# amzn/MXFusion

Hardware: AMD Instinct MI355X
Metric: ELBO-steps/sec + RBF Gram GB/s, SVGP N=65k D=8 M=1024, 1->8 MI355X (higher is better)
Workload: dtype f32; 1 GPU; SVGPRegression RBF-ARD N=65536 Q=8 M=1024, 32 MC samples (latent-input model), StochasticVariationalInference step = draw + ELBO + reverse mode + grad all-reduce + Adam; samples_per_gpu=32, parallelism=mc-samples sharded x1, 1 RCCL all-reduce of the flat gradient/step, core_precision=float64 (M x M factorisations), streaming float32

## Files before the change

mxfusion_amd/csrc/gemm_split.hip:

```cpp
#include "common.h"
#include "internal.h"
#include "split_device.h"

namespace {

typedef __bf16 bf16x8 __attribute__((ext_vector_type(8)));

constexpr int SBM = 128, SBN = 128, SNT = 256;

template <int NP>
__global__ __launch_bounds__(256) void split_planes_kernel(int64_t R, int64_t K, const float* __restrict__ X, int64_t ld,
                                                           unsigned short* __restrict__ P, int64_t pstride, const unsigned* __restrict__ maxbits) {
    __shared__ float tile[64][68];
    const int tid = threadIdx.x;
    const int64_t r0 = (int64_t)blockIdx.y * 64, k0 = (int64_t)blockIdx.x * 64;
    for (int it = 0; it < 4; ++it) {
        const int row = it * 16 + (tid >> 4), c = (tid & 15) * 4;
        const int64_t r = r0 + row, k = k0 + c;
        float4 v = make_float4(0.f, 0.f, 0.f, 0.f);
        if (r < R) {
            if (k + 3 < K && ((ld & 3) == 0) && (((uintptr_t)X & 15) == 0)) v = *reinterpret_cast<const float4*>(X + r * ld + k);
            else {
                if (k + 0 < K) v.x = X[r * ld + k + 0];
                if (k + 1 < K) v.y = X[r * ld + k + 1];
                if (k + 2 < K) v.z = X[r * ld + k + 2];
                if (k + 3 < K) v.w = X[r * ld + k + 3];
            }
        }
        tile[row][c + 0] = v.x; tile[row][c + 1] = v.y; tile[row][c + 2] = v.z; tile[row][c + 3] = v.w;
    }
    __syncthreads();
    const int row = tid & 63, kbl = tid >> 6;
    const int64_t r = r0 + row, kb = k0 / 16 + kbl;
    const int64_t Kp16 = (K + 15) / 16;
    if (r >= R || kb >= Kp16) return;
    unsigned short h[16], m[16], l[16];
    const float sc = (NP == 2 && maxbits) ? scale_from_maxbits(maxbits[0]) : 1.f;
#pragma unroll
    for (int j = 0; j < 16; ++j) {
        const float x = tile[row][kbl * 16 + j];
        if (NP == 2) {
            const float xs = x * sc;
            const _Float16 fh = (_Float16)xs;
            const _Float16 fl = (_Float16)(xs - (float)fh);
            h[j] = __builtin_bit_cast(unsigned short, fh); m[j] = __builtin_bit_cast(unsigned short, fl); l[j] = 0;
            continue;
        }
        const __bf16 bh = (__bf16)x;
        const float r1 = x - (float)bh;
        const __bf16 bm = (__bf16)r1;
        const float r2 = r1 - (float)bm;
        const __bf16 bl = (__bf16)r2;
        h[j] = __builtin_bit_cast(unsigned short, bh); m[j] = __builtin_bit_cast(unsigned short, bm); l[j] = __builtin_bit_cast(unsigned short, bl);
    }
    const int64_t off = (kb * R + r) * 16;
    auto put = [&](unsigned short* dst, const unsigned short (&v)[16]) {
        u32x4 a, b;
#pragma unroll
        for (int j = 0; j < 4; ++j) { a[j] = (unsigned)v[2 * j] | ((unsigned)v[2 * j + 1] << 16); b[j] = (unsigned)v[8 + 2 * j] | ((unsigned)v[8 + 2 * j + 1] << 16); }
        *reinterpret_cast<u32x4*>(dst) = a;
        *reinterpret_cast<u32x4*>(dst + 8) = b;
    };
    put(P + off, h);
    put(P + pstride + off, m);
    if (NP == 3) put(P + 2 * pstride + off, l);
}

__global__ __launch_bounds__(256) void maxabs_kernel(int64_t n, int64_t K, int64_t ld, const float* __restrict__ x, unsigned* __restrict__ out) {
    __shared__ unsigned wm[4];
    unsigned m = 0;
    for (int64_t i = (int64_t)blockIdx.x * 256 + threadIdx.x; i < n; i += (int64_t)gridDim.x * 256) {
        const unsigned b = __builtin_bit_cast(unsigned, x[(i / K) * ld + i % K]) & 0x7fffffffu;
        m = b > m ? b : m;
    }
    for (int o = 32; o > 0; o >>= 1) { const unsigned t = (unsigned)__shfl_xor((int)m, o); m = t > m ? t : m; }
    if ((threadIdx.x & 63) == 0) wm[threadIdx.x >> 6] = m;
    __syncthreads();
    if (threadIdx.x == 0) {
        for (int w = 1; w < 4; ++w) m = wm[w] > m ? wm[w] : m;
        atomicMax(out, m);
    }
}

__global__ __launch_bounds__(256) void maxabs_flat_kernel(int64_t n4, const uint4* __restrict__ x, unsigned* __restrict__ out) {
    __shared__ unsigned wm[4];
    unsigned m = 0;
    for (int64_t i = (int64_t)blockIdx.x * 256 + threadIdx.x; i < n4; i += (int64_t)gridDim.x * 256) {
        const uint4 v = x[i];
        const unsigned a = v.x & 0x7fffffffu, b = v.y & 0x7fffffffu, c = v.z & 0x7fffffffu, d = v.w & 0x7fffffffu;
        const unsigned ab = a > b ? a : b, cd = c > d ? c : d, q = ab > cd ? ab : cd;
        m = q > m ? q : m;
    }
    for (int o = 32; o > 0; o >>= 1) { const unsigned t = (unsigned)__shfl_xor((int)m, o); m = t > m ? t : m; }
    if ((threadIdx.x & 63) == 0) wm[threadIdx.x >> 6] = m;
    __syncthreads();
    if (threadIdx.x == 0) {
        for (int w = 1; w < 4; ++w) m = wm[w] > m ? wm[w] : m;
        atomicMax(out, m);
    }
}

struct SplitArgs {
    const unsigned short* A; const unsigned short* B; float* C;
    int64_t M, N, K16;
    int64_t pA, pB, ldc;
    float alpha, beta;
    int splitk, lower_only, atomic, nprod, use_dma;
    int c_blk;
    int64_t kchunk;
    int64_t tm, tn, ntiles, nwg;
    const float* ad0; int pow0;
    const unsigned* maxbits;
    const unsigned* maxbits2;
    unsigned* sync; int sync_n, sync_period, sync_slots;
    unsigned* maxout;
    unsigned short* Cp; int64_t pC;
    int64_t rot_div;
    int a_lower;
    int pair;
    unsigned short* Ct; int64_t pCt;
    const float* avec; float* Upart;
    int cp_nt;
};

template <bool DMA, int NP>
__global__ __launch_bounds__(SNT, (NP == 2 && !DMA) ? 4 : 3) void gemm_split_kernel(SplitArgs g) {
    constexpr int NST = (DMA && NP == 2) ? 3 : 2;
    __shared__ u32x4 smem[NST][2][NP][256];
    const int tid = threadIdx.x, lane = tid & 63, wave = tid >> 6;
    const int wm = (wave >> 1) * 64, wn = (wave & 1) * 64;
    const int64_t wid = xcd_run_item((int64_t)blockIdx.x, g.nwg);
    const int64_t split = wid / g.ntiles;
    int64_t t = wid % g.ntiles;
    int64_t tile_m, tile_n;
    if (g.lower_only) {
        int64_t row = (int64_t)((sqrt(8.0 * (double)t + 1.0) - 1.0) * 0.5);
        while (row * (row + 1) / 2 > t) --row;
        while ((row + 1) * (row + 2) / 2 <= t) ++row;
        tile_m = row; tile_n = t - row * (row + 1) / 2;
    } else {
        tile_m = t % g.tm; tile_n = t / g.tm;
    }
    const int64_t m0 = tile_m * SBM, n0 = tile_n * SBN;
    const int64_t kbeg = split * g.kchunk;
    const int64_t kend = (kbeg + g.kchunk < g.K16) ? kbeg + g.kchunk : g.K16;

    f32x16 c[2][2];
#pragma unroll
    for (int x = 0; x < 2; ++x)
#pragma unroll
        for (int y = 0; y < 2; ++y)
#pragma unroll
            for (int r = 0; r < 16; ++r) c[x][y][r] = 0.f;

    const int lrow = tid >> 1, lkh = tid & 1;
    const bool va = (m0 + lrow) < g.M, vb = (n0 + lrow) < g.N;
    const unsigned short* pa = g.A + (m0 + lrow) * 16 + lkh * 8;
    const unsigned short* pb = g.B + (n0 + lrow) * 16 + lkh * 8;
    const int sunit = lds_unit(lrow, lkh);
    u32x4 ra[NP], rb[NP];
    const u32x4 zero4 = {0u, 0u, 0u, 0u};
#define SLOAD(kb)                                                                                                                  \
    do {                                                                                                                           \
        _Pragma("unroll") for (int p = 0; p < NP; ++p) {                                                                           \
            ra[p] = va ? *reinterpret_cast<const u32x4*>(pa + p * g.pA + (kb) * g.M * 16) : zero4;                                 \
            rb[p] = vb ? *reinterpret_cast<const u32x4*>(pb + p * g.pB + (kb) * g.N * 16) : zero4;                                 \
        }                                                                                                                          \
    } while (0)
#define SSTORE(buf)                                                                                                                \
    do {                                                                                                                           \
        _Pragma("unroll") for (int p = 0; p < NP; ++p) { smem[buf][0][p][sunit] = ra[p]; smem[buf][1][p][sunit] = rb[p]; }         \
    } while (0)
    constexpr bool dma = DMA;
    const int drow = tid >> 1, dkh = (tid & 1) ^ ((drow >> 3) & 1);
    const unsigned short* da = g.A + (m0 + drow) * 16 + dkh * 8;
    const unsigned short* db = g.B + (n0 + drow) * 16 + dkh * 8;
#define SDMA(kb, buf)                                                                                                              \
    do {                                                                                                                           \
        _Pragma("unroll") for (int p = 0; p < NP; ++p) {                                                                           \
            __builtin_amdgcn_global_load_lds((const __attribute__((address_space(1))) void*)(da + p * g.pA + (kb) * g.M * 16),     \
                                             (__attribute__((address_space(3))) void*)(&smem[buf][0][p][wave * 64]), 16, 0, 0);    \
            __builtin_amdgcn_global_load_lds((const __attribute__((address_space(1))) void*)(db + p * g.pB + (kb) * g.N * 16),     \
                                             (__attribute__((address_space(3))) void*)(&smem[buf][1][p][wave * 64]), 16, 0, 0);    \
        }                                                                                                                          \
    } while (0)
    if (kbeg < kend) {
        if constexpr (dma) SDMA(kbeg, 0);
        else { SLOAD(kbeg); SSTORE(0); }
    }
    if constexpr (NST == 3) {
        if (kbeg + 1 < kend) {
            SDMA(kbeg + 1, 1);
            __builtin_amdgcn_s_waitcnt(0xF70 | (2 * NP));
        } else {
            __builtin_amdgcn_s_waitcnt(0xF70);
        }
        __builtin_amdgcn_s_barrier();
    } else {
        __syncthreads();
    }
    const int li = lane & 31, lk = lane >> 5;
    int ua[2], ub[2];
#pragma unroll
    for (int x = 0; x < 2; ++x) { ua[x] = lds_unit(wm + 32 * x + li, lk); ub[x] = lds_unit(wn + 32 * x + li, lk); }
    int cur = 0;
    for (int64_t kb = kbeg; kb < kend; ++kb) {
        const bool more = kb + 1 < kend;
        if constexpr (NST == 3) {
            if (kb + 2 < kend) SDMA(kb + 2, (cur + 2) % 3);
        } else {
            if (more) { if constexpr (dma) SDMA(kb + 1, cur ^ 1); else SLOAD(kb + 1); }
        }
        u32x4 a[2][NP], b[2][NP];
#pragma unroll
        for (int x = 0; x < 2; ++x)
#pragma unroll
            for (int p = 0; p < NP; ++p) {
                a[x][p] = smem[cur][0][p][ua[x]];
                b[x][p] = smem[cur][1][p][ub[x]];
            }
#pragma unroll
        for (int x = 0; x < 2; ++x)
#pragma unroll
            for (int y = 0; y < 2; ++y) {
                f32x16 acc = c[x][y];
                if constexpr (NP == 3) {
#define BF(v) __builtin_bit_cast(bf16x8, v)
                    if (g.nprod >= 6) {
                        acc = __builtin_amdgcn_mfma_f32_32x32x16_bf16(BF(a[x][1]), BF(b[y][1]), acc, 0, 0, 0);
                        acc = __builtin_amdgcn_mfma_f32_32x32x16_bf16(BF(a[x][0]), BF(b[y][2]), acc, 0, 0, 0);
                        acc = __builtin_amdgcn_mfma_f32_32x32x16_bf16(BF(a[x][2]), BF(b[y][0]), acc, 0, 0, 0);
                    }
                    acc = __builtin_amdgcn_mfma_f32_32x32x16_bf16(BF(a[x][0]), BF(b[y][1]), acc, 0, 0, 0);
                    acc = __builtin_amdgcn_mfma_f32_32x32x16_bf16(BF(a[x][1]), BF(b[y][0]), acc, 0, 0, 0);
                    acc = __builtin_amdgcn_mfma_f32_32x32x16_bf16(BF(a[x][0]), BF(b[y][0]), acc, 0, 0, 0);
#undef BF
                } else {
#define HF(v) __builtin_bit_cast(f16x8, v)
                    if (g.nprod >= 3) {
                        acc = __builtin_amdgcn_mfma_f32_32x32x16_f16(HF(a[x][0]), HF(b[y][1]), acc, 0, 0, 0);
                        acc = __builtin_amdgcn_mfma_f32_32x32x16_f16(HF(a[x][1]), HF(b[y][0]), acc, 0, 0, 0);
                    }
                    acc = __builtin_amdgcn_mfma_f32_32x32x16_f16(HF(a[x][0]), HF(b[y][0]), acc, 0, 0, 0);
#undef HF
                }
                c[x][y] = acc;
            }
        if constexpr (NST == 3) {
            asm volatile("" ::: "memory");
            if (kb + 2 < kend) __builtin_amdgcn_s_waitcnt(0xF70 | (2 * NP));
            else __builtin_amdgcn_s_waitcnt(0xF70);
            __builtin_amdgcn_s_barrier();
            asm volatile("" ::: "memory");
            cur = cur == 2 ? 0 : cur + 1;
        } else {
            if constexpr (!dma) { if (more) SSTORE(cur ^ 1); }
            __syncthreads();
            cur ^= 1;
        }
    }
#undef SLOAD
#undef SSTORE
#undef SDMA
    float alpha = g.alpha;
    const float beta = g.beta;
    if (g.ad0) { const float v = g.ad0[0]; for (int i = 0; i < g.pow0; ++i) alpha *= v; }
    if (g.maxbits) alpha /= scale_from_maxbits(g.maxbits[0]);
    if (g.maxbits2) alpha /= scale_from_maxbits(g.maxbits2[0]);
    const bool atomic = g.atomic != 0;
#pragma unroll
    for (int x = 0; x < 2; ++x)
#pragma unroll
        for (int y = 0; y < 2; ++y)
#pragma unroll
            for (int r = 0; r < 16; ++r) {
                const int64_t row = m0 + wm + x * 32 + (r & 3) + 8 * (r >> 2) + 4 * (lane >> 5);
                const int64_t col = n0 + wn + y * 32 + (lane & 31);
                if (row < g.M && col < g.N && !(g.lower_only && col > row)) {
                    float* p = g.c_blk ? g.C + ((col >> 4) * g.M + row) * 16 + (col & 15) : g.C + row * g.ldc + col;
                    const float v = alpha * c[x][y][r];
                    if (atomic) atomic_add(p, v);
                    else *p = (beta == 0.f) ? v : v + beta * (*p);
                }
            }
}

constexpr int WBN = 256;

__device__ __forceinline__ u32x4 gload16(unsigned voff, const void* sbase) {
    u32x4 r;
    asm volatile("global_load_dwordx4 %0, %1, %2" : "=v"(r) : "v"(voff), "s"(sbase) : "memory");
    return r;
}
__device__ __forceinline__ u32x4 gload16_o1024(unsigned voff, const void* sbase) {
    u32x4 r;
    asm volatile("global_load_dwordx4 %0, %1, %2 offset:1024" : "=v"(r) : "v"(voff), "s"(sbase) : "memory");
    return r;
}

template <int NH, bool LSKIP = false, bool CPL = false>
__device__ __forceinline__ void wide_body(const SplitArgs& g) {
    constexpr int XT = 4;
    constexpr int WBMt = 32 * XT * NH;
    constexpr int NU = 64 * XT * NH;
    constexpr int ND = XT / 4;
    constexpr int NTH = 256 * NH;
    __shared__ u32x4 smem[3][2][NU];
    const int tid = threadIdx.x, lane = tid & 63, wave = tid >> 6, wq = wave & 3, wh = wave >> 2;
    int patience = 2;
    float cmax = 0.f;
    const int nsub = (CPL && g.pair) ? 2 : 1;
    for (int64_t wid0 = blockIdx.x; wid0 < g.nwg; wid0 += gridDim.x)
    for (int sub = 0; sub < nsub; ++sub) {
    const int64_t wid = xcd_run_item(wid0, g.nwg);
    const int64_t split = wid / g.ntiles;
    int64_t t = wid % g.ntiles;
    int64_t tile_m, tile_n;
    if (g.lower_only) {
        int64_t row = 0;
        while (t >= (WBMt * row + WBMt - 1) / WBN + 1) { t -= (WBMt * row + WBMt - 1) / WBN + 1; ++row; }
        tile_m = row; tile_n = t;
    } else {
        tile_m = t % g.tm; tile_n = t / g.tm;
        if constexpr (CPL) {
            if (g.pair) {
                const int64_t role = t % g.tm, sp = t / g.tm;
                tile_n = 2 * sp + sub;
                tile_m = sub ? g.tm - 1 - role : role;
                if (tile_n >= g.tn) break;
            } else if (g.a_lower && g.rot_div > 0) tile_m = (tile_m + tile_n / g.rot_div) % g.tm;
        }
    }
    const int64_t m0 = tile_m * WBMt, n0 = tile_n * WBN;
    const int64_t kbeg = split * g.kchunk;
    int64_t kend = (kbeg + g.kchunk < g.K16) ? kbeg + g.kchunk : g.K16;
    if constexpr (CPL) { if (g.a_lower) { const int64_t kl = (m0 + WBMt + 15) / 16; kend = kl < kend ? kl : kend; } }
    const bool kdesc = CPL && g.pair && sub == 1;
    const int64_t korg = kdesc ? kend - 1 : kbeg, kdir = kdesc ? -1 : 1, nk = kend - kbeg;
#define KMAP(i) (korg + kdir * (i))
    if (g.sync && g.sync_period == 0 && sub == 0) wg_rendezvous(g.sync + wid / g.sync_n, (unsigned)g.sync_n, patience);

    f32x16 c[XT][2];
#pragma unroll
    for (int x = 0; x < XT; ++x)
#pragma unroll
        for (int y = 0; y < 2; ++y)
#pragma unroll
            for (int r = 0; r < 16; ++r) c[x][y][r] = 0.f;

    const int drow = tid >> 1, dkh = (tid & 1) ^ ((drow >> 3) & 1);
    const unsigned short* da = g.A + (m0 + drow) * 16 + dkh * 8;
    const unsigned bvoff = (unsigned)(((64 * wq + (lane & 31)) * 16 + (lane >> 5) * 8) * 2);
    const unsigned short* bbase = g.B + n0 * 16;
    const int li = lane & 31, lk = lane >> 5;
    int ua[XT];
#pragma unroll
    for (int x = 0; x < XT; ++x) ua[x] = lds_unit(32 * XT * wh + 32 * x + li, lk);

    u32x4 b0[2][2], b1[2][2], b2[2][2];
#define W_ISSUE(kb, SLOT, BR)                                                                                                       \
    do {                                                                                                                            \
        const unsigned short* bk_ = bbase + (kb) * g.N * 16;                                                                        \
        BR[0][0] = gload16(bvoff, bk_);                                                                                             \
        BR[1][0] = gload16_o1024(bvoff, bk_);                                                                                       \
        BR[0][1] = gload16(bvoff, bk_ + g.pB);                                                                                      \
        BR[1][1] = gload16_o1024(bvoff, bk_ + g.pB);                                                                                \
        _Pragma("unroll") for (int u_ = 0; u_ < ND; ++u_) {                                                                         \
            __builtin_amdgcn_global_load_lds((const __attribute__((address_space(1))) void*)(da + u_ * (NTH / 2) * 16 + (kb) * g.M * 16), \
                                             (__attribute__((address_space(3))) void*)(&smem[SLOT][0][wave * 64 + NTH * u_]), 16, 0, 0); \
            __builtin_amdgcn_global_load_lds((const __attribute__((address_space(1))) void*)(da + u_ * (NTH / 2) * 16 + g.pA + (kb) * g.M * 16), \
                                             (__attribute__((address_space(3))) void*)(&smem[SLOT][1][wave * 64 + NTH * u_]), 16, 0, 0); \
        }                                                                                                                           \
    } while (0)
#define W_WAIT_ASM(NSTR, BR)                                                                                                        \
    do {                                                                                                                            \
        asm volatile("s_waitcnt vmcnt(" NSTR ")" : "+v"(BR[0][0]), "+v"(BR[0][1]), "+v"(BR[1][0]), "+v"(BR[1][1])::"memory");      \
    } while (0)
#define W_WAIT1(BR)                                                                                                                 \
    do {                                                                                                                            \
        W_WAIT_ASM("6", BR);                                                                                                        \
        __builtin_amdgcn_s_barrier();                                                                                               \
        asm volatile("" ::: "memory");                                                                                              \
    } while (0)
#define W_WAIT0(BR)                                                                                                                 \
    do {                                                                                                                            \
        W_WAIT_ASM("0", BR);                                                                                                        \
        __builtin_amdgcn_s_barrier();                                                                                               \
        asm volatile("" ::: "memory");                                                                                              \
    } while (0)
#define HF(v) __builtin_bit_cast(f16x8, v)
#define WMMA(a, b, c) __builtin_amdgcn_mfma_f32_32x32x16_f16(HF(a), HF(b), c, 0, 0, 0)
#define W_COMPUTE(SLOT, BR)                                                                                                         \
    do {                                                                                                                            \
        u32x4 a_[XT][2];                                                                                                            \
        _Pragma("unroll") for (int x = 0; x < XT; ++x) { a_[x][0] = smem[SLOT][0][ua[x]]; a_[x][1] = smem[SLOT][1][ua[x]]; }         \
        W_MFMAS(a_, BR);                                                                                                            \
    } while (0)
#define W_MFMAS(a_, BR)                                                                                                             \
    do {                                                                                                                            \
        _Pragma("unroll") for (int x = 0; x < XT; ++x)                                                                              \
            _Pragma("unroll") for (int y = 0; y < 2; ++y)                                                                           \
                c[x][y] = WMMA(BR[y][0], a_[x][1], c[x][y]);                                                            \
        _Pragma("unroll") for (int x = 0; x < XT; ++x)                                                                              \
            _Pragma("unroll") for (int y = 0; y < 2; ++y)                                                                           \
                c[x][y] = WMMA(BR[y][1], a_[x][0], c[x][y]);                                                            \
        _Pragma("unroll") for (int x = 0; x < XT; ++x)                                                                              \
            _Pragma("unroll") for (int y = 0; y < 2; ++y)                                                                           \
                c[x][y] = WMMA(BR[y][0], a_[x][0], c[x][y]);                                                            \
    } while (0)
#define W_STEP(kk, SLOT, BR, SLOT2, BR2, BRN)                                                                                       \
    do {                                                                                                                            \
        const int64_t i2_ = (kk) + 2 < nk ? (kk) + 2 : nk - 1;                                                                      \
        const int64_t k2_ = KMAP(i2_);                                                                                              \
        W_ISSUE(k2_, SLOT2, BR2);                                                                                                   \
        W_COMPUTE(SLOT, BR);                                                                                                        \
        W_WAIT1(BRN);                                                                                                               \
    } while (0)
    bool idle = false;
    if constexpr (LSKIP) idle = g.lower_only && (m0 + 32 * XT * wh + 32 * XT - 1) < (n0 + 64 * wq);
    if (LSKIP && idle) {
        if (kbeg < kend) {
#define W_ISSUE_A(kb, SLOT)                                                                                                         \
            do {                                                                                                                    \
                _Pragma("unroll") for (int u_ = 0; u_ < ND; ++u_) {                                                                 \
                    __builtin_amdgcn_global_load_lds((const __attribute__((address_space(1))) void*)(da + u_ * (NTH / 2) * 16 + (kb) * g.M * 16), \
                                                     (__attribute__((address_space(3))) void*)(&smem[SLOT][0][wave * 64 + NTH * u_]), 16, 0, 0); \
                    __builtin_amdgcn_global_load_lds((const __attribute__((address_space(1))) void*)(da + u_ * (NTH / 2) * 16 + g.pA + (kb) * g.M * 16), \
                                                     (__attribute__((address_space(3))) void*)(&smem[SLOT][1][wave * 64 + NTH * u_]), 16, 0, 0); \
                }                                                                                                                   \
            } while (0)
#define W_WAITL(NSTR) do { asm volatile("s_waitcnt vmcnt(" NSTR ")" ::: "memory"); __builtin_amdgcn_s_barrier(); asm volatile("" ::: "memory"); } while (0)
            const int64_t klast = kend - 1;
            int64_t kb = kbeg;
            for (int i = (int)((kend - kbeg) % 3); i > 0; --i, ++kb) {
                W_ISSUE_A(kb, 0);
                W_WAITL("0");
                __builtin_amdgcn_s_barrier();
            }
            if (kb < kend) {
                W_ISSUE_A(kb, 0);
                W_ISSUE_A(kb + 1, 1);
                W_WAITL("2");
                int trip = 0, sync_ix = 0;
                for (; kb < kend; kb += 3) {
#pragma unroll
                    for (int s3 = 0; s3 < 3; ++s3) {
                        const int64_t k2_ = kb + s3 + 2 < kend ? kb + s3 + 2 : klast;
                        if (s3 == 0) W_ISSUE_A(k2_, 2); else if (s3 == 1) W_ISSUE_A(k2_, 0); else W_ISSUE_A(k2_, 1);
                        W_WAITL("2");
                    }
                    if (g.sync_period > 0 && ++trip == g.sync_period) {
                        trip = 0;
                        if (sync_ix < g.sync_slots) wg_rendezvous(g.sync + split * g.sync_slots + sync_ix, (unsigned)g.sync_n, patience);
                        ++sync_ix;
                    }
                }
                asm volatile("s_waitcnt vmcnt(0)" ::: "memory");
            }
#undef W_WAITL
#undef W_ISSUE_A
        }
    } else
    if (nk > 0) {
        int64_t kb = 0;
        for (int i = (int)(nk % 3); i > 0; --i, ++kb) {
            W_ISSUE(KMAP(kb), 0, b0);
            W_WAIT0(b0);
            W_COMPUTE(0, b0);
            __builtin_amdgcn_s_barrier();
        }
        if (kb < nk) {
            W_ISSUE(KMAP(kb), 0, b0);
            W_ISSUE(KMAP(kb + 1), 1, b1);
            W_WAIT1(b0);
            int trip = 0, sync_ix = 0;
            for (; kb < nk; kb += 3) {
                W_STEP(kb, 0, b0, 2, b2, b1);
                W_STEP(kb + 1, 1, b1, 0, b0, b2);
                W_STEP(kb + 2, 2, b2, 1, b1, b0);
                if (g.sync_period > 0 && ++trip == g.sync_period) {
                    trip = 0;
                    if (sync_ix < g.sync_slots) wg_rendezvous(g.sync + split * g.sync_slots + sync_ix, (unsigned)g.sync_n, patience);
                    ++sync_ix;
                }
            }
            asm volatile("s_waitcnt vmcnt(0)" : "+v"(b0[0][0]), "+v"(b0[0][1]), "+v"(b0[1][0]), "+v"(b0[1][1]), "+v"(b1[0][0]), "+v"(b1[0][1]),
                         "+v"(b1[1][0]), "+v"(b1[1][1])::"memory");
        }
    }
#undef KMAP
#undef W_STEP
#undef W_MFMAS
#undef WMMA
#undef HF
#undef W_WAIT1
#undef W_WAIT0
#undef W_WAIT_ASM
#undef W_ISSUE
    float alpha = g.alpha;
    const float beta = g.beta;
    if (g.ad0) { const float v = g.ad0[0]; for (int i = 0; i < g.pow0; ++i) alpha *= v; }
    if (g.maxbits) alpha /= scale_from_maxbits(g.maxbits[0]);
    if (g.maxbits2) alpha /= scale_from_maxbits(g.maxbits2[0]);
    const bool atomic = g.atomic != 0;
    if constexpr (CPL) {
        float* alds = reinterpret_cast<float*>(reinterpret_cast<unsigned short*>(&smem[0][0][0]) + (NTH / 64) * (32 * 68));
        float aval = 0.f;
        if (g.Ct && g.avec && tid < WBMt) aval = g.avec[m0 + tid];
#pragma unroll
        for (int x = 0; x < XT; ++x) {
            const int64_t row = m0 + 32 * XT * wh + 32 * x + li;
#pragma unroll
            for (int y = 0; y < 2; ++y)
#pragma unroll
                for (int q = 0; q < 4; q += 2) {
                    unsigned hi[4], lo[4];
#pragma unroll
                    for (int d = 0; d < 4; ++d) {
                        const f32x2 v = {alpha * c[x][y][4 * q + 2 * d], alpha * c[x][y][4 * q + 2 * d + 1]};
                        const f16x2 fh = __builtin_convertvector(v, f16x2);
                        const f16x2 fl = __builtin_convertvector(v - __builtin_convertvector(fh, f32x2), f16x2);
                        hi[d] = __builtin_bit_cast(unsigned, fh); lo[d] = __builtin_bit_cast(unsigned, fl);
                    }
#pragma unroll
                    for (int d = 0; d < 2; ++d) {
                        asm volatile("s_nop 1\n\tv_permlane32_swap_b32 %0, %1\n\ts_nop 1" : "+v"(hi[d]), "+v"(hi[2 + d]));
                        asm volatile("s_nop 1\n\tv_permlane32_swap_b32 %0, %1\n\ts_nop 1" : "+v"(lo[d]), "+v"(lo[2 + d]));
                    }
                    const int64_t col = n0 + 64 * wq + 32 * y + 8 * (q + lk);
                    unsigned short* p = g.Cp + ((col >> 4) * g.M + row) * 16 + (col & 15);
                    const u32x4 vh = {hi[0], hi[1], hi[2], hi[3]}, vl = {lo[0], lo[1], lo[2], lo[3]};
                    if (g.cp_nt & 1) { __builtin_nontemporal_store(vh, reinterpret_cast<u32x4*>(p)); __builtin_nontemporal_store(vl, reinterpret_cast<u32x4*>(p + g.pC)); }
                    else { *reinterpret_cast<u32x4*>(p) = vh; *reinterpret_cast<u32x4*>(p + g.pC) = vl; }
                }
        }
        if (g.Ct) {
            constexpr int RS = 68;
            asm volatile("" ::: "memory"); __builtin_amdgcn_s_barrier(); asm volatile("" ::: "memory");
            unsigned short* wl = reinterpret_cast<unsigned short*>(&smem[0][0][0]) + wave * (32 * RS);
            if (g.avec) {
                if (tid < WBMt) alds[tid] = aval;
                asm volatile("s_waitcnt lgkmcnt(0)" ::: "memory"); __builtin_amdgcn_s_barrier(); asm volatile("" ::: "memory");
            }
            const int nn = lane >> 1, hh = lane & 1;
            float ua[2] = {0.f, 0.f};
#pragma unroll
            for (int x = 0; x < XT; ++x) {
                const int64_t mrow = m0 + 32 * XT * wh + 32 * x;
#pragma unroll
                for (int pl = 0; pl < 2; ++pl) {
#pragma unroll
                    for (int y = 0; y < 2; ++y)
#pragma unroll
                        for (int q = 0; q < 4; ++q) {
                            unsigned w2[2];
#pragma unroll
                            for (int d = 0; d < 2; ++d) {
                                const f32x2 v = {alpha * c[x][y][4 * q + 2 * d], alpha * c[x][y][4 * q + 2 * d + 1]};
                                const f16x2 fh = __builtin_convertvector(v, f16x2);
                                const f16x2 fo = pl == 0 ? fh : __builtin_convertvector(v - __builtin_convertvector(fh, f32x2), f16x2);
                                w2[d] = __builtin_bit_cast(unsigned, fo);
                            }
                            const u32x2 wv = {w2[0], w2[1]};
                            *reinterpret_cast<u32x2*>(wl + li * RS + 32 * y + 8 * q + 4 * lk) = wv;
                        }
                    __builtin_amdgcn_fence(__ATOMIC_SEQ_CST, "wavefront");
                    __builtin_amdgcn_wave_barrier();
#pragma unroll
                    for (int nh = 0; nh < 2; ++nh)
#pragma unroll
                        for (int mb = 0; mb < 2; ++mb) {
                            unsigned short e[8];
#pragma unroll
                            for (int j = 0; j < 8; ++j) e[j] = wl[(16 * mb + 8 * hh + j) * RS + 32 * nh + nn];
                            if (g.avec) {
                                const f32x4 a0 = *reinterpret_cast<const f32x4*>(alds + 32 * XT * wh + 32 * x + 16 * mb + 8 * hh);
                                const f32x4 a1 = *reinterpret_cast<const f32x4*>(alds + 32 * XT * wh + 32 * x + 16 * mb + 8 * hh + 4);
#pragma unroll
                                for (int j = 0; j < 4; ++j) {
                                    ua[nh] = fmaf(a0[j], (float)__builtin_bit_cast(_Float16, e[j]), ua[nh]);
                                    ua[nh] = fmaf(a1[j], (float)__builtin_bit_cast(_Float16, e[4 + j]), ua[nh]);
                                }
                            }
                            const u32x4 ov = {(unsigned)e[0] | ((unsigned)e[1] << 16), (unsigned)e[2] | ((unsigned)e[3] << 16),
                                              (unsigned)e[4] | ((unsigned)e[5] << 16), (unsigned)e[6] | ((unsigned)e[7] << 16)};
                            const int64_t n = n0 + 64 * wq + 32 * nh + nn;
                            unsigned short* p = g.Ct + (int64_t)pl * g.pCt + (((mrow >> 4) + mb) * g.N + n) * 16 + 8 * hh;
                            if (g.cp_nt & 2) __builtin_nontemporal_store(ov, reinterpret_cast<u32x4*>(p)); else *reinterpret_cast<u32x4*>(p) = ov;
                        }
                    __builtin_amdgcn_fence(__ATOMIC_SEQ_CST, "wavefront");
                    __builtin_amdgcn_wave_barrier();
                }
            }
            if (g.avec) {
#pragma unroll
                for (int nh = 0; nh < 2; ++nh) {
                    const float t2 = ua[nh] + __shfl_xor(ua[nh], 1, 64);
                    if (hh == 0) g.Upart[((m0 + 32 * XT * wh) >> 7) * g.N + n0 + 64 * wq + 32 * nh + nn] = t2;
                }
            }
            asm volatile("s_waitcnt lgkmcnt(0)" ::: "memory"); __builtin_amdgcn_s_barrier(); asm volatile("" ::: "memory");
        }
    } else
#pragma unroll
    for (int x = 0; x < XT; ++x) {
        const int64_t row = m0 + 32 * XT * wh + 32 * x + li;
#pragma unroll
        for (int y = 0; y < 2; ++y)
#pragma unroll
            for (int q = 0; q < 4; ++q) {
                const int64_t col = n0 + 64 * wq + 32 * y + 8 * q + 4 * lk;
                float* p = g.c_blk ? g.C + ((col >> 4) * g.M + row) * 16 + (col & 15) : g.C + row * g.ldc + col;
                f32x4 v = {alpha * c[x][y][4 * q], alpha * c[x][y][4 * q + 1], alpha * c[x][y][4 * q + 2], alpha * c[x][y][4 * q + 3]};
                if (g.lower_only && col + 3 > row) {
#pragma unroll
                    for (int e = 0; e < 4; ++e)
                        if (col + e <= row) { if (atomic) atomic_add(p + e, v[e]); else p[e] = (beta == 0.f) ? v[e] : v[e] + beta * p[e]; }
                } else if (atomic) {
#pragma unroll
                    for (int e = 0; e < 4; ++e) atomic_add(p + e, v[e]);
                } else if (beta == 0.f) {
                    *reinterpret_cast<f32x4*>(p) = v;
                    if (g.maxout) cmax = fmaxf(fmaxf(cmax, fmaxf(fabsf(v[0]), fabsf(v[1]))), fmaxf(fabsf(v[2]), fabsf(v[3])));
                } else {
                    const f32x4 o = *reinterpret_cast<const f32x4*>(p);
                    *reinterpret_cast<f32x4*>(p) = v + beta * o;
                }
            }
    }
    }
    if (g.maxout) {
#pragma unroll
        for (int o = 32; o > 0; o >>= 1) cmax = fmaxf(cmax, __shfl_xor(cmax, o, 64));
        if (lane == 0 && __builtin_bit_cast(unsigned, cmax) > *(volatile unsigned*)g.maxout) atomicMax(g.maxout, __builtin_bit_cast(unsigned, cmax));
    }
}

__global__ __launch_bounds__(256, 2) void gemm_f16x2_wide_kernel_128(SplitArgs g) { wide_body<1>(g); }
__global__ __launch_bounds__(512, 2) void gemm_f16x2_wide_kernel_256(SplitArgs g) { wide_body<2>(g); }
__global__ __launch_bounds__(512, 2) void gemm_f16x2_wide_kernel_256lo(SplitArgs g) { wide_body<2, true>(g); }
__global__ __launch_bounds__(512, 2) void gemm_f16x2_wide_kernel_256pl(SplitArgs g) { wide_body<2, false, true>(g); }
__global__ __launch_bounds__(256, 2) void gemm_f16x2_wide_kernel_128pl(SplitArgs g) { wide_body<1, false, true>(g); }

__global__ void split_scale_kernel(float* C, int64_t M, int64_t N, int64_t ldc, float beta, int lower_only) {
    const int64_t col = (int64_t)blockIdx.x * 256 + threadIdx.x, row = blockIdx.y;
    if (col < N && !(lower_only && col > row)) {
        float* p = C + row * ldc + col;
        *p = (beta == 0.f) ? 0.f : beta * (*p);
    }
}

}

size_t mxf_split_plane_elems(int64_t R, int64_t K) { return (size_t)((K + 15) / 16) * (size_t)R * 16; }

int mxf_maxabs_internal(mxf_ctx* h, int64_t R, int64_t K, const float* x, int64_t ld, unsigned* out, hipStream_t st, bool zero) {
    if (zero) MXF_HIP(h, hipMemsetAsync(out, 0, sizeof(unsigned), st));
    const int64_t n = R * K;
    if (n <= 0) return 0;
    int64_t nb = (n + 256 * 16 - 1) / (256 * 16);
    if (ld == K && n % 4 == 0 && ((uintptr_t)x % 16) == 0 && n >= (int64_t)1 << 22) {
        if (nb > 2048) nb = 2048;
        hipLaunchKernelGGL(maxabs_flat_kernel, dim3((unsigned)nb), dim3(256), 0, st, n / 4, reinterpret_cast<const uint4*>(x), out);
        MXF_LAUNCH_CHECK(h);
        return 0;
    }
    if (nb > 256) nb = 256;
    hipLaunchKernelGGL(maxabs_kernel, dim3((unsigned)nb), dim3(256), 0, st, n, K, ld, x, out);
    MXF_LAUNCH_CHECK(h);
    return 0;
}

int mxf_split_planes_internal(mxf_ctx* h, int64_t R, int64_t K, const float* X, int64_t ld, unsigned short* planes, hipStream_t st, int mode,
                              const unsigned* maxbits) {
    if (R <= 0 || K <= 0) return 0;
    const int64_t pstride = (int64_t)mxf_split_plane_elems(R, K);
    dim3 grid((unsigned)((K + 63) / 64), (unsigned)((R + 63) / 64));
    if (grid.y > 65535u) MXF_FAIL(h, -3, "split planes: too many rows for one launch (%lld)", (long long)R);
    if (mode == MXF_SPLIT_F16X2) hipLaunchKernelGGL(split_planes_kernel<2>, grid, dim3(256), 0, st, R, K, X, ld, planes, pstride, maxbits);
    else hipLaunchKernelGGL(split_planes_kernel<3>, grid, dim3(256), 0, st, R, K, X, ld, planes, pstride, (const unsigned*)nullptr);
    MXF_LAUNCH_CHECK(h);
    return 0;
}

namespace {

enum SplitKernel { SK_WIDE_256PL, SK_WIDE_128PL, SK_WIDE_256LO, SK_WIDE_256, SK_WIDE_128, SK_TILE_DMA_F16, SK_TILE_F16, SK_TILE_DMA_BF16, SK_TILE_BF16 };

struct SplitPlan { SplitArgs g; SplitKernel kernel; unsigned grid, block, ncounters; bool prescale; };

int split_check_output(mxf_ctx* h, int mode, int64_t M, int64_t N, const MxfSplitOut& o) {
    if (o.planes && o.C) MXF_FAIL(h, -2, "mxf_gemm_split: one output, C or planes");
    if ((o.planes_t && !o.planes) || (o.avec && (!o.planes_t || !o.Upart))) MXF_FAIL(h, -2, "mxf_gemm_split: the transposed planes come with the planes output, the partial sums with both");
    if (o.planes && (mode != MXF_SPLIT_F16X2 || (M % 128) != 0 || (N % WBN) != 0 || o.beta != 0.0 || o.lower_only || o.blocked))
        MXF_FAIL(h, -2, "mxf_gemm_split: the planes output needs the f16x2 format, M %% 128 == 0, N %% 256 == 0, beta == 0 and a full product");
    if (!o.planes && o.a_lower) MXF_FAIL(h, -2, "mxf_gemm_split: a_lower is implemented for the planes output only");
    if (o.blocked && (N % 16 != 0 || o.beta != 0.0 || o.lower_only || o.ldc != N)) MXF_FAIL(h, -2, "mxf_gemm_split: the blocked output layout needs N %% 16 == 0, ldc == N, beta == 0 and a full product");
    if (o.lower_only && (M + SBM - 1) / SBM != (N + SBN - 1) / SBN) MXF_FAIL(h, -2, "mxf_gemm_split: lower_only needs a square output");
    return 0;
}

void split_plan_wide(SplitPlan& p, int64_t rows, int reserve_cus) {
    SplitArgs& g = p.g;
    const bool planes = g.c_blk == 2;
    const int64_t tm = g.tm, splitk = g.splitk;
    static const int64_t wide_grid_env = MXF_KNOB("MXF_SPLIT_WIDE_GRID", 0);
    int64_t wide_grid = wide_grid_env > 0 ? wide_grid_env : (planes ? (256 - reserve_cus) / 8 * 8 : 256) * (rows == 256 ? 1 : 2);
    if (g.pair && wide_grid / 8 >= tm) wide_grid = (wide_grid / 8) / tm * tm * 8;
    const int64_t grid = (wide_grid >= 8 && g.nwg > wide_grid) ? wide_grid / 8 * 8 : g.nwg;
    p.grid = (unsigned)grid;
    static const int sync_period_env = (int)MXF_KNOB("MXF_SPLIT_SYNC_PERIOD", 16);
    if (planes && g.a_lower) {
        if (!g.pair) g.rot_div = (grid / 8) / tm > 0 ? (grid / 8) / tm : 1;
    } else if (!g.lower_only && splitk == 1) {
        if (strip_rendezvous_ok(tm, g.nwg, grid)) { p.ncounters = (unsigned)(g.nwg / tm); g.sync_n = (int)tm; }
    } else if (splitk > 1 && g.nwg <= grid && g.ntiles >= 2 && sync_period_env > 0) {
        const int64_t trips = g.kchunk / 3;
        int64_t period = sync_period_env;
        int64_t slots_per = trips / period;
        while (slots_per * splitk > (int64_t)(MXF_NRING / 8)) { period *= 2; slots_per = trips / period; }
        if (slots_per >= 1) {
            p.ncounters = (unsigned)(slots_per * splitk);
            g.sync_n = (int)g.ntiles; g.sync_period = (int)period; g.sync_slots = (int)slots_per;
        }
    }
}

int split_plan(mxf_ctx* h, int mode, int64_t M, int64_t N, int64_t K, const MxfSplitScale& sc, const MxfPlanes& A, const MxfPlanes& B,
               const MxfSplitOut& o, const MxfSplitSched& sched, SplitPlan& p) {
    const int rc = split_check_output(h, mode, M, N, o);
    if (rc) return rc;
    const bool planes = o.planes != nullptr, f16 = mode == MXF_SPLIT_F16X2, lower = o.lower_only != 0;
    SplitArgs& g = p.g;
    g.A = A.p; g.pA = A.stride; g.maxbits = A.maxbits; g.B = B.p; g.pB = B.stride; g.maxbits2 = B.maxbits;
    g.M = M; g.N = N; g.K16 = (K + 15) / 16;
    g.alpha = (float)sc.alpha; g.ad0 = sc.ad0; g.pow0 = sc.pow0;
    g.C = o.C; g.ldc = planes ? N : o.ldc; g.beta = (float)o.beta; g.lower_only = o.lower_only; g.c_blk = planes ? 2 : o.blocked;
    g.Cp = o.planes; g.pC = o.pstride; g.a_lower = o.a_lower; g.Ct = o.planes_t; g.pCt = o.pstride_t; g.avec = o.avec; g.Upart = o.Upart;
    g.nprod = 6; g.use_dma = 1; g.cp_nt = 0;
    const bool wide = planes || ((lower || o.blocked) && f16 && (M % 128) == 0 && (N % WBN) == 0 && (o.ldc % 4) == 0 && (((uintptr_t)o.C) % 16) == 0 &&
                                 (!lower || M == N));
    const int64_t rows = wide && (M % 256) == 0 ? 256 : 128, cols = wide ? WBN : SBN;
    const bool dma = (M % SBM) == 0 && (N % SBN) == 0;
    if (wide) p.kernel = rows == 256 ? (planes ? SK_WIDE_256PL : lower ? SK_WIDE_256LO : SK_WIDE_256) : (planes ? SK_WIDE_128PL : SK_WIDE_128);
    else p.kernel = f16 ? (dma ? SK_TILE_DMA_F16 : SK_TILE_F16) : (dma ? SK_TILE_DMA_BF16 : SK_TILE_BF16);
    p.block = wide ? (unsigned)(2 * rows) : (unsigned)SNT;
    const int64_t tm = (M + rows - 1) / rows, tn = (N + cols - 1) / cols;
    int64_t tiles = lower ? 0 : tm * tn;
    for (int64_t r = 0; lower && r < tm; ++r) tiles += (rows * r + rows - 1) / cols + 1;
    const int64_t cus = 256 - sched.reserve_cus;
    const int64_t slots = cus * (!wide ? (f16 ? 4 : 3) : sched.reserve_cus >= 128 ? 4 : rows == 256 ? 1 : 2);
    int64_t sk = 1;
    if (tiles < slots && g.K16 >= 16 && !planes) {
        sk = slots / tiles;
        if (sk * tiles < (slots * 3) / 4) sk = (2 * slots) / tiles;
        if (sk > g.K16 / 8) sk = g.K16 / 8;
    }
    const int64_t kchunk = g.K16 > sk ? (g.K16 + (int)sk - 1) / (int)sk : 1;
    const int splitk = g.K16 > kchunk ? (int)((g.K16 + kchunk - 1) / kchunk) : 1;
    g.splitk = splitk; g.kchunk = kchunk; g.atomic = splitk > 1;
    g.tm = tm; g.tn = tn; g.ntiles = tiles; g.nwg = tiles * splitk;
    g.pair = (planes && o.a_lower && tm >= 2 && tn >= 2) ? 1 : 0;
    if (g.pair) { g.ntiles = tm * ((tn + 1) / 2); g.nwg = g.ntiles; }
    if (g.nwg > 2147483647LL) MXF_FAIL(h, -3, "mxf_gemm_split: grid too large");
    p.prescale = g.atomic && o.beta != 1.0;
    if (p.prescale && M > 65535) MXF_FAIL(h, -3, "mxf_gemm_split: split-K path needs M<=65535");
    g.sync = nullptr; g.sync_n = 1; g.sync_period = 0; g.sync_slots = 0; g.rot_div = 0; g.maxout = nullptr;
    p.ncounters = 0; p.grid = (unsigned)g.nwg;
    if (wide) {
        g.maxout = (splitk == 1 && o.beta == 0.0 && !lower) ? o.maxout : nullptr;
        split_plan_wide(p, rows, sched.reserve_cus);
    }
    return 0;
}

int split_launch(mxf_ctx* h, hipStream_t st, SplitPlan& p) {
    SplitArgs& g = p.g;
    if (p.prescale)
        hipLaunchKernelGGL(split_scale_kernel, dim3((unsigned)((g.N + 255) / 256), (unsigned)g.M), dim3(256), 0, st, g.C, g.M, g.N, g.ldc, g.beta, g.lower_only);
    if (p.ncounters) g.sync = mxf_gsync(h, p.ncounters);
    if (!g.sync) { g.sync_n = 1; g.sync_period = 0; g.sync_slots = 0; }
    static void (*const kernels[])(SplitArgs) = {
        gemm_f16x2_wide_kernel_256pl, gemm_f16x2_wide_kernel_128pl, gemm_f16x2_wide_kernel_256lo, gemm_f16x2_wide_kernel_256, gemm_f16x2_wide_kernel_128,
        gemm_split_kernel<true, 2>, gemm_split_kernel<false, 2>, gemm_split_kernel<true, 3>, gemm_split_kernel<false, 3>};
    hipLaunchKernelGGL(kernels[p.kernel], dim3(p.grid), dim3(p.block), 0, st, g);
    MXF_LAUNCH_CHECK(h);
    return 0;
}

}

int mxf_gemm_split_internal(mxf_ctx* h, hipStream_t st, int mode, int64_t M, int64_t N, int64_t K, MxfSplitScale scale, MxfPlanes A, MxfPlanes B,
                            MxfSplitOut out, MxfSplitSched sched) {
    if (M <= 0 || N <= 0) return 0;
    SplitPlan p;
    const int rc = split_plan(h, mode, M, N, K, scale, A, B, out, sched, p);
    return rc ? rc : split_launch(h, st, p);
}

extern "C" int mxf_gemm_f32x3(mxf_handle h, int64_t M, int64_t N, int64_t K, double alpha, const void* A, int64_t lda, const void* B,
                              int64_t ldb, double beta, void* C, int64_t ldc, int lower_only, void* stream) {
    if (!h) return -1;
    if (M <= 0 || N <= 0 || K <= 0) MXF_FAIL(h, -2, "mxf_gemm_f32x3: bad shape");
    if (!A || !B || !C) MXF_FAIL(h, -2, "mxf_gemm_f32x3: null argument");
    hipStream_t st = (hipStream_t)stream;
    const size_t ea = mxf_split_plane_elems(M, K), eb = mxf_split_plane_elems(N, K);
    const size_t need = mxf_align(3 * ea * 2) + mxf_align(3 * eb * 2);
    char* ws = (char*)mxf_ws(h, need);
    if (!ws) MXF_FAIL(h, -4, "mxf_gemm_f32x3: cannot allocate %zu bytes of scratch", need);
    unsigned short* pa = (unsigned short*)ws;
    unsigned short* pb = (unsigned short*)(ws + mxf_align(3 * ea * 2));
    int rc = mxf_split_planes_internal(h, M, K, (const float*)A, lda, pa, st);
    if (rc) return rc;
    rc = mxf_split_planes_internal(h, N, K, (const float*)B, ldb, pb, st);
    if (rc) return rc;
    return mxf_gemm_split_internal(h, st, MXF_SPLIT_BF16X3, M, N, K, {.alpha = alpha}, {pa, (int64_t)ea}, {pb, (int64_t)eb},
                                   {.C = (float*)C, .ldc = ldc, .beta = beta, .lower_only = lower_only});
}

extern "C" int mxf_gemm_f16x2(mxf_handle h, int64_t M, int64_t N, int64_t K, double alpha, const void* A, int64_t lda, const void* B,
                              int64_t ldb, double beta, void* C, int64_t ldc, int lower_only, void* stream) {
    if (!h) return -1;
    if (M <= 0 || N <= 0 || K <= 0) MXF_FAIL(h, -2, "mxf_gemm_f16x2: bad shape");
    if (!A || !B || !C) MXF_FAIL(h, -2, "mxf_gemm_f16x2: null argument");
    hipStream_t st = (hipStream_t)stream;
    const size_t ea = mxf_split_plane_elems(M, K), eb = mxf_split_plane_elems(N, K);
    const size_t need = mxf_align(2 * ea * 2) + mxf_align(2 * eb * 2) + mxf_align(2 * sizeof(unsigned));
    char* ws = (char*)mxf_ws(h, need);
    if (!ws) MXF_FAIL(h, -4, "mxf_gemm_f16x2: cannot allocate %zu bytes of scratch", need);
    unsigned short* pa = (unsigned short*)ws;
    unsigned short* pb = (unsigned short*)(ws + mxf_align(2 * ea * 2));
    unsigned* mx = (unsigned*)(ws + mxf_align(2 * ea * 2) + mxf_align(2 * eb * 2));
    int rc = mxf_maxabs_internal(h, M, K, (const float*)A, lda, mx, st);
    if (rc) return rc;
    rc = mxf_maxabs_internal(h, N, K, (const float*)B, ldb, mx + 1, st);
    if (rc) return rc;
    rc = mxf_split_planes_internal(h, M, K, (const float*)A, lda, pa, st, MXF_SPLIT_F16X2, mx);
    if (rc) return rc;
    rc = mxf_split_planes_internal(h, N, K, (const float*)B, ldb, pb, st, MXF_SPLIT_F16X2, mx + 1);
    if (rc) return rc;
    return mxf_gemm_split_internal(h, st, MXF_SPLIT_F16X2, M, N, K, {.alpha = alpha}, {pa, (int64_t)ea, mx}, {pb, (int64_t)eb, mx + 1},
                                   {.C = (float*)C, .ldc = ldc, .beta = beta, .lower_only = lower_only});
}

extern "C" int mxf_f16x2_split(mxf_handle h, int64_t R, int64_t K, const void* X, int64_t ld, void* planes, void* maxword, void* stream) {
    if (!h) return -1;
    if (R <= 0 || K <= 0 || !X || !planes || !maxword) MXF_FAIL(h, -2, "mxf_f16x2_split: bad argument");
    int rc = mxf_maxabs_internal(h, R, K, (const float*)X, ld, (unsigned*)maxword, (hipStream_t)stream);
    if (rc) return rc;
    return mxf_split_planes_internal(h, R, K, (const float*)X, ld, (unsigned short*)planes, (hipStream_t)stream, MXF_SPLIT_F16X2, (const unsigned*)maxword);
}

extern "C" int mxf_gemm_f16x2_planes(mxf_handle h, int64_t M, int64_t N, int64_t K, double alpha, const void* A_planes, const void* A_maxword,
                                     const void* B_planes, const void* B_maxword, double beta, void* C, int64_t ldc, int lower_only, void* stream) {
    if (!h) return -1;
    if (M <= 0 || N <= 0 || K <= 0 || !A_planes || !B_planes || !A_maxword || !B_maxword || !C) MXF_FAIL(h, -2, "mxf_gemm_f16x2_planes: bad argument");
    const int blocked = lower_only == 2;
    return mxf_gemm_split_internal(h, (hipStream_t)stream, MXF_SPLIT_F16X2, M, N, K, {.alpha = alpha},
                                   {(const unsigned short*)A_planes, (int64_t)mxf_split_plane_elems(M, K), (const unsigned*)A_maxword},
                                   {(const unsigned short*)B_planes, (int64_t)mxf_split_plane_elems(N, K), (const unsigned*)B_maxword},
                                   {.C = (float*)C, .ldc = blocked ? N : ldc, .beta = beta, .lower_only = blocked ? 0 : lower_only, .blocked = blocked});
}

extern "C" int64_t mxf_f32x3_plane_elems(int64_t R, int64_t K) { return (R > 0 && K > 0) ? (int64_t)mxf_split_plane_elems(R, K) : 0; }

extern "C" int mxf_f32x3_split(mxf_handle h, int64_t R, int64_t K, const void* X, int64_t ld, void* planes, void* stream) {
    if (!h) return -1;
    if (R <= 0 || K <= 0 || !X || !planes) MXF_FAIL(h, -2, "mxf_f32x3_split: bad argument");
    return mxf_split_planes_internal(h, R, K, (const float*)X, ld, (unsigned short*)planes, (hipStream_t)stream);
}

extern "C" int mxf_gemm_f32x3_planes(mxf_handle h, int64_t M, int64_t N, int64_t K, double alpha, const void* A_planes, const void* B_planes,
                                     double beta, void* C, int64_t ldc, int lower_only, void* stream) {
    if (!h) return -1;
    if (M <= 0 || N <= 0 || K <= 0 || !A_planes || !B_planes || !C) MXF_FAIL(h, -2, "mxf_gemm_f32x3_planes: bad argument");
    return mxf_gemm_split_internal(h, (hipStream_t)stream, MXF_SPLIT_BF16X3, M, N, K, {.alpha = alpha},
                                   {(const unsigned short*)A_planes, (int64_t)mxf_split_plane_elems(M, K)},
                                   {(const unsigned short*)B_planes, (int64_t)mxf_split_plane_elems(N, K)},
                                   {.C = (float*)C, .ldc = ldc, .beta = beta, .lower_only = lower_only});
}
```

Measured before the change: 45.06 ELBO-steps/sec.

## Add symmetric split-K kernel for lower-only A·Aᵀ Gram products

Adds a symmetric variant of the 256-row lower-only wide kernel for the case where A and B are the same matrix. Off-diagonal tiles are computed once on strictly-lower blocks, and diagonal tiles use a single-plane product computed in two sub-passes whose results are mirrored via atomics. Diagonal tiles get a longer K chunk. This aims to skip the redundant second-plane loads and cross products that symmetry makes unnecessary, and to rebalance split-K work across CUs. The cost is more atomic traffic on diagonal tiles and a more complex schedule.

```diff
diff --git a/mxfusion_amd/csrc/gemm_split.hip b/mxfusion_amd/csrc/gemm_split.hip
--- a/mxfusion_amd/csrc/gemm_split.hip
+++ b/mxfusion_amd/csrc/gemm_split.hip
@@ -1,6 +1,7 @@
 #include "common.h"
 #include "internal.h"
 #include "split_device.h"
+#include "split_sym_plan.h"
 
 namespace {
 
@@ -121,6 +122,7 @@
     unsigned short* Ct; int64_t pCt;
     const float* avec; float* Upart;
     int cp_nt;
+    int64_t sy_kchunk;
 };
 
 template <bool DMA, int NP>
@@ -298,8 +300,9 @@
     return r;
 }
 
-template <int NH, bool LSKIP = false, bool CPL = false>
+template <int NH, bool LSKIP = false, bool CPL = false, bool SY = false>
 __device__ __forceinline__ void wide_body(const SplitArgs& g) {
+    static_assert(!SY || (NH == 2 && LSKIP && !CPL), "the symmetric form is a 256-row lower-only kernel");
     constexpr int XT = 4;
     constexpr int WBMt = 32 * XT * NH;
     constexpr int NU = 64 * XT * NH;
@@ -309,13 +312,27 @@
     const int tid = threadIdx.x, lane = tid & 63, wave = tid >> 6, wq = wave & 3, wh = wave >> 2;
     int patience = 2;
     float cmax = 0.f;
-    const int nsub = (CPL && g.pair) ? 2 : 1;
+    const int nsub = SY ? 2 : (CPL && g.pair) ? 2 : 1;
     for (int64_t wid0 = blockIdx.x; wid0 < g.nwg; wid0 += gridDim.x)
     for (int sub = 0; sub < nsub; ++sub) {
     const int64_t wid = xcd_run_item(wid0, g.nwg);
-    const int64_t split = wid / g.ntiles;
-    int64_t t = wid % g.ntiles;
+    int64_t split, t, kchunk = g.kchunk;
+    if constexpr (!SY) { split = wid / g.ntiles; t = wid % g.ntiles; }
     int64_t tile_m, tile_n;
+    bool diag = false;
+    if constexpr (SY) {
+        const int64_t noff = g.ntiles * g.splitk;
+        diag = wid >= noff;
+        if (diag) {
+            split = (wid - noff) / g.tm; tile_m = tile_n = (wid - noff) % g.tm; kchunk = g.sy_kchunk;
+        } else {
+            if (sub == 1) break;
+            split = wid / g.ntiles; t = wid % g.ntiles;
+            int64_t row = 1;
+            while (t >= row) { t -= row; ++row; }
+            tile_m = row; tile_n = t;
+        }
+    } else
     if (g.lower_only) {
         int64_t row = 0;
         while (t >= (WBMt * row + WBMt - 1) / WBN + 1) { t -= (WBMt * row + WBMt - 1) / WBN + 1; ++row; }
@@ -332,8 +349,8 @@
         }
     }
     const int64_t m0 = tile_m * WBMt, n0 = tile_n * WBN;
-    const int64_t kbeg = split * g.kchunk;
-    int64_t kend = (kbeg + g.kchunk < g.K16) ? kbeg + g.kchunk : g.K16;
+    const int64_t kbeg = split * kchunk;
+    int64_t kend = (kbeg + kchunk < g.K16) ? kbeg + kchunk : g.K16;
     if constexpr (CPL) { if (g.a_lower) { const int64_t kl = (m0 + WBMt + 15) / 16; kend = kl < kend ? kl : kend; } }
     const bool kdesc = CPL && g.pair && sub == 1;
     const int64_t korg = kdesc ? kend - 1 : kbeg, kdir = kdesc ? -1 : 1, nk = kend - kbeg;
@@ -416,8 +433,39 @@
         W_COMPUTE(SLOT, BR);                                                                                                        \
         W_WAIT1(BRN);                                                                                                               \
     } while (0)
+#define D_ISSUE(kb, SLOT, BR)                                                                                                       \
+    do {                                                                                                                            \
+        const unsigned short* bk_ = bsel + (kb) * g.N * 16;                                                                         \
+        BR[0][0] = gload16(bvoff, bk_);                                                                                             \
+        BR[1][0] = gload16_o1024(bvoff, bk_);                                                                                       \
+        _Pragma("unroll") for (int u_ = 0; u_ < ND; ++u_)                                                                           \
+            __builtin_amdgcn_global_load_lds((const __attribute__((address_space(1))) void*)(da + u_ * (NTH / 2) * 16 + (kb) * g.M * 16), \
+                                             (__attribute__((address_space(3))) void*)(&smem[SLOT][0][wave * 64 + NTH * u_]), 16, 0, 0); \
+    } while (0)
+#define D_WAIT(NSTR, BR)                                                                                                            \
+    do {                                                                                                                            \
+        asm volatile("s_waitcnt vmcnt(" NSTR ")" : "+v"(BR[0][0]), "+v"(BR[1][0])::"memory");                                      \
+        __builtin_amdgcn_s_barrier();                                                                                               \
+        asm volatile("" ::: "memory");                                                                                              \
+    } while (0)
+#define D_COMPUTE(SLOT, BR)                                                                                                         \
+    do {                                                                                                                            \
+        u32x4 a_[XT];                                                                                                               \
+        _Pragma("unroll") for (int x = 0; x < XT; ++x) a_[x] = smem[SLOT][0][ua[x]];                                                \
+        _Pragma("unroll") for (int x = 0; x < XT; ++x)                                                                              \
+            _Pragma("unroll") for (int y = 0; y < 2; ++y)                                                                           \
+                c[x][y] = WMMA(BR[y][0], a_[x], c[x][y]);                                                                           \
+    } while (0)
+#define D_STEP(kk, SLOT, BR, SLOT2, BR2, BRN)                                                                                       \
+    do {                                                                                                                            \
+        const int64_t i2_ = (kk) + 2 < nk ? (kk) + 2 : nk - 1;                                                                      \
+        D_ISSUE(kbeg + i2_, SLOT2, BR2);                                                                                            \
+        D_COMPUTE(SLOT, BR);                                                                                                        \
+        D_WAIT("3", BRN);                                                                \
+    } while (0)
     bool idle = false;
-    if constexpr (LSKIP) idle = g.lower_only && (m0 + 32 * XT * wh + 32 * XT - 1) < (n0 + 64 * wq);
+    if constexpr (LSKIP && !SY) idle = g.lower_only && (m0 + 32 * XT * wh + 32 * XT - 1) < (n0 + 64 * wq);
+    if constexpr (SY) idle = diag && sub == 1 && (m0 + 32 * XT * wh + 32 * XT - 1) < (n0 + 64 * wq);
     if (LSKIP && idle) {
         if (kbeg < kend) {
 #define W_ISSUE_A(kb, SLOT)                                                                                                         \
@@ -425,11 +473,13 @@
                 _Pragma("unroll") for (int u_ = 0; u_ < ND; ++u_) {                                                                 \
                     __builtin_amdgcn_global_load_lds((const __attribute__((address_space(1))) void*)(da + u_ * (NTH / 2) * 16 + (kb) * g.M * 16), \
                                                      (__attribute__((address_space(3))) void*)(&smem[SLOT][0][wave * 64 + NTH * u_]), 16, 0, 0); \
+                    if constexpr (!SY)                        \
                     __builtin_amdgcn_global_load_lds((const __attribute__((address_space(1))) void*)(da + u_ * (NTH / 2) * 16 + g.pA + (kb) * g.M * 16), \
                                                      (__attribute__((address_space(3))) void*)(&smem[SLOT][1][wave * 64 + NTH * u_]), 16, 0, 0); \
                 }                                                                                                                   \
             } while (0)
-#define W_WAITL(NSTR) do { asm volatile("s_waitcnt vmcnt(" NSTR ")" ::: "memory"); __builtin_amdgcn_s_barrier(); asm volatile("" ::: "memory"); } while (0)
+#define W_WAITL_(NSTR) do { asm volatile("s_waitcnt vmcnt(" NSTR ")" ::: "memory"); __builtin_amdgcn_s_barrier(); asm volatile("" ::: "memory"); } while (0)
+#define W_WAITL(NSTR) do { if constexpr (SY && (NSTR)[0] == '2') W_WAITL_("1"); else W_WAITL_(NSTR); } while (0)
             const int64_t klast = kend - 1;
             int64_t kb = kbeg;
             for (int i = (int)((kend - kbeg) % 3); i > 0; --i, ++kb) {
@@ -449,7 +499,7 @@
                         if (s3 == 0) W_ISSUE_A(k2_, 2); else if (s3 == 1) W_ISSUE_A(k2_, 0); else W_ISSUE_A(k2_, 1);
                         W_WAITL("2");
                     }
-                    if (g.sync_period > 0 && ++trip == g.sync_period) {
+                    if (!SY && g.sync_period > 0 && ++trip == g.sync_period) {
                         trip = 0;
                         if (sync_ix < g.sync_slots) wg_rendezvous(g.sync + split * g.sync_slots + sync_ix, (unsigned)g.sync_n, patience);
                         ++sync_ix;
@@ -458,7 +508,31 @@
                 asm volatile("s_waitcnt vmcnt(0)" ::: "memory");
             }
 #undef W_WAITL
+#undef W_WAITL_
 #undef W_ISSUE_A
+        }
+    } else
+    if (SY && diag) {
+        if (nk > 0) {
+            const unsigned short* bsel = sub == 0 ? bbase + g.pB : bbase;
+            int64_t kb = 0;
+            for (int i = (int)(nk % 3); i > 0; --i, ++kb) {
+                D_ISSUE(kbeg + kb, 0, b0);
+                D_WAIT("0", b0);
+                D_COMPUTE(0, b0);
+                __builtin_amdgcn_s_barrier();
+            }
+            if (kb < nk) {
+                D_ISSUE(kbeg + kb, 0, b0);
+                D_ISSUE(kbeg + kb + 1, 1, b1);
+                D_WAIT("3", b0);
+                for (; kb < nk; kb += 3) {
+                    D_STEP(kb, 0, b0, 2, b2, b1);
+                    D_STEP(kb + 1, 1, b1, 0, b0, b2);
+                    D_STEP(kb + 2, 2, b2, 1, b1, b0);
+                }
+                asm volatile("s_waitcnt vmcnt(0)" : "+v"(b0[0][0]), "+v"(b0[1][0]), "+v"(b1[0][0]), "+v"(b1[1][0])::"memory");
+            }
         }
     } else
     if (nk > 0) {
@@ -489,6 +563,10 @@
         }
     }
 #undef KMAP
+#undef D_STEP
+#undef D_COMPUTE
+#undef D_WAIT
+#undef D_ISSUE
 #undef W_STEP
 #undef W_MFMAS
 #undef WMMA
@@ -503,6 +581,24 @@
     if (g.maxbits) alpha /= scale_from_maxbits(g.maxbits[0]);
     if (g.maxbits2) alpha /= scale_from_maxbits(g.maxbits2[0]);
     const bool atomic = g.atomic != 0;
+    if (SY && diag && sub == 0) {
+#pragma unroll
+        for (int x = 0; x < XT; ++x) {
+            const int64_t row = m0 + 32 * XT * wh + 32 * x + li;
+#pragma unroll
+            for (int y = 0; y < 2; ++y)
+#pragma unroll
+                for (int q = 0; q < 4; ++q)
+#pragma unroll
+                    for (int e = 0; e < 4; ++e) {
+                        const int64_t col = n0 + 64 * wq + 32 * y + 8 * q + 4 * lk + e;
+                        const float v = alpha * c[x][y][4 * q + e];
+                        if (col < row) atomic_add(g.C + row * g.ldc + col, v);
+                        else if (col > row) atomic_add(g.C + col * g.ldc + row, v);
+                        else atomic_add(g.C + row * g.ldc + row, v + v);
+                    }
+        }
+    } else
     if constexpr (CPL) {
         float* alds = reinterpret_cast<float*>(reinterpret_cast<unsigned short*>(&smem[0][0][0]) + (NTH / 64) * (32 * 68));
         float aval = 0.f;
@@ -639,6 +735,7 @@
 __global__ __launch_bounds__(256, 2) void gemm_f16x2_wide_kernel_128(SplitArgs g) { wide_body<1>(g); }
 __global__ __launch_bounds__(512, 2) void gemm_f16x2_wide_kernel_256(SplitArgs g) { wide_body<2>(g); }
 __global__ __launch_bounds__(512, 2) void gemm_f16x2_wide_kernel_256lo(SplitArgs g) { wide_body<2, true>(g); }
+__global__ __launch_bounds__(512, 2) void gemm_f16x2_wide_kernel_256sy(SplitArgs g) { wide_body<2, true, false, true>(g); }
 __global__ __launch_bounds__(512, 2) void gemm_f16x2_wide_kernel_256pl(SplitArgs g) { wide_body<2, false, true>(g); }
 __global__ __launch_bounds__(256, 2) void gemm_f16x2_wide_kernel_128pl(SplitArgs g) { wide_body<1, false, true>(g); }
 
@@ -685,7 +782,7 @@
 
 namespace {
 
-enum SplitKernel { SK_WIDE_256PL, SK_WIDE_128PL, SK_WIDE_256LO, SK_WIDE_256, SK_WIDE_128, SK_TILE_DMA_F16, SK_TILE_F16, SK_TILE_DMA_BF16, SK_TILE_BF16 };
+enum SplitKernel { SK_WIDE_256PL, SK_WIDE_128PL, SK_WIDE_256LO, SK_WIDE_256SY, SK_WIDE_256, SK_WIDE_128, SK_TILE_DMA_F16, SK_TILE_F16, SK_TILE_DMA_BF16, SK_TILE_BF16 };
 
 struct SplitPlan { SplitArgs g; SplitKernel kernel; unsigned grid, block, ncounters; bool prescale; };
 
@@ -758,8 +855,13 @@
     }
     const int64_t kchunk = g.K16 > sk ? (g.K16 + (int)sk - 1) / (int)sk : 1;
     const int splitk = g.K16 > kchunk ? (int)((g.K16 + kchunk - 1) / kchunk) : 1;
-    g.splitk = splitk; g.kchunk = kchunk; g.atomic = splitk > 1;
+    g.splitk = splitk; g.kchunk = kchunk; g.atomic = splitk > 1; g.sy_kchunk = 0;
     g.tm = tm; g.tn = tn; g.ntiles = tiles; g.nwg = tiles * splitk;
+    if (p.kernel == SK_WIDE_256LO && g.atomic && M == N && A.p == B.p && A.stride == B.stride) {
+        const MxfSymSplit s = mxf_sym_split_plan(g.K16, tm, slots);
+        p.kernel = SK_WIDE_256SY;
+        g.ntiles = s.n_off; g.splitk = (int)s.s_off; g.kchunk = s.n_off ? s.c_off : 1; g.sy_kchunk = s.c_diag; g.nwg = s.items();
+    }
     g.pair = (planes && o.a_lower && tm >= 2 && tn >= 2) ? 1 : 0;
     if (g.pair) { g.ntiles = tm * ((tn + 1) / 2); g.nwg = g.ntiles; }
     if (g.nwg > 2147483647LL) MXF_FAIL(h, -3, "mxf_gemm_split: grid too large");
@@ -781,7 +883,8 @@
     if (p.ncounters) g.sync = mxf_gsync(h, p.ncounters);
     if (!g.sync) { g.sync_n = 1; g.sync_period = 0; g.sync_slots = 0; }
     static void (*const kernels[])(SplitArgs) = {
-        gemm_f16x2_wide_kernel_256pl, gemm_f16x2_wide_kernel_128pl, gemm_f16x2_wide_kernel_256lo, gemm_f16x2_wide_kernel_256, gemm_f16x2_wide_kernel_128,
+        gemm_f16x2_wide_kernel_256pl, gemm_f16x2_wide_kernel_128pl, gemm_f16x2_wide_kernel_256lo, gemm_f16x2_wide_kernel_256sy, gemm_f16x2_wide_kernel_256,
+        gemm_f16x2_wide_kernel_128,
         gemm_split_kernel<true, 2>, gemm_split_kernel<false, 2>, gemm_split_kernel<true, 3>, gemm_split_kernel<false, 3>};
     hipLaunchKernelGGL(kernels[p.kernel], dim3(p.grid), dim3(p.block), 0, st, g);
     MXF_LAUNCH_CHECK(h);
diff --git a/mxfusion_amd/csrc/split_sym_plan.h b/mxfusion_amd/csrc/split_sym_plan.h
--- /dev/null
+++ b/mxfusion_amd/csrc/split_sym_plan.h
@@ -0,0 +1,30 @@
+#pragma once
+#include <stdint.h>
+
+struct MxfSymSplit {
+    int64_t n_off, n_diag;
+    int64_t s_off, c_off;
+    int64_t s_diag, c_diag;
+    int64_t items() const { return n_off * s_off + n_diag * s_diag; }
+};
+
+inline MxfSymSplit mxf_sym_split_plan(int64_t K16, int64_t tm, int64_t slots) {
+    MxfSymSplit s = {};
+    s.n_off = tm * (tm - 1) / 2; s.n_diag = tm;
+    const auto ceil_div = [](int64_t a, int64_t b) { return (a + b - 1) / b; };
+    if (s.n_off == 0) {
+        int64_t sd = slots < K16 / 12 ? slots : K16 / 12;
+        if (sd < 1) sd = 1;
+        s.c_diag = ceil_div(K16, sd); s.s_diag = ceil_div(K16, s.c_diag);
+        return s;
+    }
+    int64_t so = (3 * slots) / (3 * s.n_off + 2 * s.n_diag);
+    if (so > K16 / 8) so = K16 / 8;
+    if (so < 1) so = 1;
+    for (;; --so) {
+        s.c_off = ceil_div(K16, so); s.c_diag = (3 * s.c_off + 1) / 2;
+        s.s_off = ceil_div(K16, s.c_off); s.s_diag = ceil_div(K16, s.c_diag);
+        if (s.items() <= slots || so == 1) break;
+    }
+    return s;
+}
```

Measured after the change: 41.38 ELBO-steps/sec. 8.2% lower.
